# pkhungurn/talking-head-anime-4-demo

Hardware: NVIDIA H100
Metric: 512x512 RGBA frames/sec (higher is better)
Workload: dtype f16/tf32 operands (10-bit mantissa), f32 accumulate, f32 storage outside conv operands

## Files before the change

tha4_b200/csrc/conv_halo.cu:

```cuda
#include "conv.cuh"
#include "profiler.cuh"
#include "conv_tc_device.cuh"
#include <cuda.h>
#include <cstring>
#include <map>
#include <mutex>
#include <tuple>

namespace tha4 {
static long long* g_dbg_buf = nullptr;

namespace {

using namespace tc;
using namespace tcdev;

constexpr int HT_W = 8, HT_H = 16;
constexpr int HALO_W = HT_W + 2;
__host__ __device__ constexpr int halo_h(int wg) { return HT_H * wg + 2; }
__host__ __device__ constexpr int halo_rows(int wg) { return HALO_W * halo_h(wg); }
__host__ __device__ constexpr int halo_a_bytes(int rowb, int wg) { return ((halo_rows(wg) * rowb + 1023) / 1024) * 1024; }
__host__ __device__ constexpr int halo_threads(int wg) { return 128 * wg + 32; }
static_assert((HT_H * HALO_W * 64) % 1024 == 0, "second warpgroup's halo offset keeps the swizzle phase");

__host__ __device__ constexpr int halo_min_ctas(int bn, int sa, int cs, int op, int wg) {
    return wg > 1 ? (bn <= 32 ? 2 : 1) : cs > 1 || bn >= 128 ? 1 : ((sa == (op == OP_F16N ? 2 : 1) && bn <= 32) ? 4 : 2);
}
template <int BN, int SA, int SB, int CS, int OP, int XF, int WG>
__global__ void __launch_bounds__(halo_threads(WG), halo_min_ctas(BN, SA, CS, OP, WG)) conv_halo_kernel(const __grid_constant__ CUtensorMap tmA, const __grid_constant__ CUtensorMap tmB,
                                                                const __grid_constant__ CUtensorMap tmO32, const __grid_constant__ CUtensorMap tmO16,
                                                                const __grid_constant__ CUtensorMap tmR, const TcParams p) {
    static_assert(OP != OP_TF32, "halo kernel: f16 operands");
    static_assert(BN <= 128, "the accumulator of one warpgroup: BN registers per thread");
    static_assert(WG == 1 || (WG == 2 && CS == 1 && BN <= 64), "two consumer warpgroups: unsplit launches, two accumulators of at most 64 columns");
    constexpr int ROWB = op_row_bytes(OP);
    constexpr int KCE = op_kch(OP);
    constexpr int HALO_ROWS = halo_rows(WG);
    constexpr int A_BYTES = halo_a_bytes(ROWB, WG);
    constexpr int B_BYTES = BN * ROWB;
    constexpr int PRODUCER_WARP = 4 * WG;
    constexpr int EPI_BYTES = (int)(((size_t)SA * A_BYTES + (size_t)SB * B_BYTES) / WG) & ~1023;
    constexpr int NSLOT = CS == 1 ? epi_nslot(BN, EPI_BYTES) : 0;
    extern __shared__ uint8_t smem_raw[];
    uint8_t* smem = smem_raw + ((1024u - (tc::smem_u32(smem_raw) & 1023u)) & 1023u);
    uint8_t* smA = smem;
    uint8_t* smB = smem + SA * A_BYTES;
    uint64_t* bars = reinterpret_cast<uint64_t*>(smB + SB * B_BYTES);
    uint64_t* a_full = bars, *a_empty = bars + SA;
    uint64_t* b_full = bars + 2 * SA, *b_empty = b_full + SB;
    uint64_t* res_bars = b_empty + SB;
    float* xf_A = reinterpret_cast<float*>(reinterpret_cast<uint8_t*>(res_bars + 4 * WG) + ((16u - (tc::smem_u32(res_bars + 4 * WG) & 15u)) & 15u));

    const int warp = threadIdx.x >> 5, lane = threadIdx.x & 31;
    const bool dbg_on = p.dbg != nullptr && (blockIdx.x % 97) == 0 && blockIdx.y == 0 && (blockIdx.x / 97) * CS + blockIdx.z < 32;
    long long* dbg = dbg_on ? p.dbg + ((blockIdx.x / 97) * CS + blockIdx.z) * 32 : nullptr;
#define HSTAMP(role, i) do { if (dbg) dbg[(role) * 8 + (i)] = clock64(); } while (0)
    if (threadIdx.x == 0) HSTAMP(0, 0);
    int tile = blockIdx.x;
    const int tx = tile % p.tiles_x; tile /= p.tiles_x;
    const int ty = tile % p.tiles_y;
    const int n = tile / p.tiles_y;
    const int x0 = tx * HT_W, y0 = ty * (HT_H * WG);
    const int n0 = blockIdx.y * BN;
    const int split = blockIdx.z;
    const int c_per = (p.cpt + CS - 1) / CS;
    const int cb0 = split * c_per;
    const int nc = max(0, min(p.cpt, cb0 + c_per) - cb0);
    const int nb = nc * 9;

    if (threadIdx.x == 0) {
        for (int s = 0; s < SA; ++s) { mbar_init(smem_u32(a_full + s), 1); mbar_init(smem_u32(a_empty + s), 128 * WG); }
        for (int s = 0; s < SB; ++s) { mbar_init(smem_u32(b_full + s), 1); mbar_init(smem_u32(b_empty + s), 128 * WG); }
        for (int s = 0; s < 4 * WG; ++s) mbar_init(smem_u32(res_bars + s), 1);
        asm volatile("fence.mbarrier_init.release.cluster;\n" ::: "memory");
        asm volatile("prefetch.tensormap [%0];\n" :: "l"(&tmA) : "memory");
        asm volatile("prefetch.tensormap [%0];\n" :: "l"(&tmB) : "memory");
    }
    __syncthreads();
    if (threadIdx.x == 0) HSTAMP(0, 1);
    pdl_trigger();
    const int npre = p.pre_b ? min(nb, SB) : 0;
    if (warp == PRODUCER_WARP && lane == 0) {
        for (int i = 0; i < npre; ++i) {
            const uint32_t full = smem_u32(b_full + i);
            mbar_expect_tx(full, B_BYTES);
            tma_load_3d(smem_u32(smB + i * B_BYTES), &tmB, (cb0 + i / 9) * KCE, n0, i % 9, full);
        }
    }
    pdl_wait();
    if (threadIdx.x == 0) HSTAMP(0, 2);

    Acc<BN> acc;
    if (nc > 0) {
        if (warp == PRODUCER_WARP) {
            if (lane == 0) {
                int bi = 0;
                for (int ci = 0; ci < nc; ++ci) {
                    const int sa = ci % SA;
                    mbar_wait(smem_u32(a_empty + sa), ((ci / SA) & 1) ^ 1);
                    mbar_expect_tx(smem_u32(a_full + sa), HALO_ROWS * ROWB);
                    tma_load_4d(smem_u32(smA + sa * A_BYTES), &tmA, (cb0 + ci) * KCE, x0 - 1, y0 - 1, n, smem_u32(a_full + sa));
                    for (int tap = 0; tap < 9; ++tap, ++bi) {
                        if (bi < npre) continue;
                        const int sb = bi % SB;
                        mbar_wait(smem_u32(b_empty + sb), ((bi / SB) & 1) ^ 1);
                        mbar_expect_tx(smem_u32(b_full + sb), B_BYTES);
                        tma_load_3d(smem_u32(smB + sb * B_BYTES), &tmB, (cb0 + ci) * KCE, n0, tap, smem_u32(b_full + sb));
                    }
                }
            }
        } else {
            const int te = threadIdx.x;
            const int wg = WG == 1 ? 0 : te >> 7;
            constexpr int XBAR = WG == 1 ? 1 : 3;
            __half* hA = reinterpret_cast<__half*>(xf_A);
            __half* hB = hA + p.xf_C;
            const bool silu = p.xf_act == ACT_SILU || p.xf_act == ACT_SILU_FAST;
            if (XF) {
                double2* chs = reinterpret_cast<double2*>(xf_A + 2 * p.xf_C);
                xf_build_coef<128 * WG, XBAR>(p, n, te, hA, hB, chs, cb0 * KCE, (cb0 + nc) * KCE);
                if (te == 0) HSTAMP(2, 0);
            }
// ... 5 lines not shown
                if (XF) {
                    const int c0 = (cb0 + ci) * KCE;
                    constexpr int HC = ROWB / 32;
                    for (int it = te; it < 2 * HALO_ROWS; it += 128 * WG) {
                        const int row = it >> 1, half = it & 1;
                        const int hy = row / HALO_W, hx = row - hy * HALO_W;
                        const int iy = y0 - 1 + hy, ix = x0 - 1 + hx;
                        if (iy < 0 || iy >= p.inH || ix < 0 || ix >= p.inW) continue;
                        const int swz = ROWB == 128 ? (row & 7) : ((row >> 1) & 3);
                        xf_chunks<HC>(smA + sa * A_BYTES + row * ROWB, swz, half * HC, c0, p, hA, hB, silu);
                    }
                    asm volatile("fence.proxy.async.shared::cta;\n" ::: "memory");
                    asm volatile("bar.sync %0, %1;\n" :: "n"(XBAR), "n"(128 * WG) : "memory");
                    if (te == 0 && ci == nc - 1) HSTAMP(2, 2);
                }
                const uint32_t a_base = smem_u32(smA + sa * A_BYTES) + (uint32_t)(wg * HT_H * HALO_W * ROWB);
#pragma unroll
                for (int tap = 0; tap < 9; ++tap, ++bi) {
                    const int sb = bi % SB;
                    mbar_wait(smem_u32(b_full + sb), (bi / SB) & 1);
                    const int shift = (p.dy[0][tap] + 1) * HALO_W + (p.dx[0][tap] + 1);
                    const uint32_t a0 = a_base + shift * ROWB, a1 = a0 + 8 * HALO_W * ROWB;
                    const uint32_t b_addr = smem_u32(smB + sb * B_BYTES);
                    wg_fence();
#pragma unroll
                    for (int k = 0; k < ROWB / 32; ++k) {
                        const uint64_t bd = make_smem_desc_sw<ROWB>(b_addr + 32 * k);
                        const uint32_t accum = (ci > 0 || tap > 0 || k > 0) ? 1u : 0u;
                        Wgmma<BN>::f16(acc.d[0], make_desc_sbo<ROWB>(a0 + 32 * k, HALO_W * ROWB), bd, accum);
                        Wgmma<BN>::f16(acc.d[1], make_desc_sbo<ROWB>(a1 + 32 * k, HALO_W * ROWB), bd, accum);
                    }
                    wg_commit();
                    if (tap < 8) {
                        wg_wait<1>();
                        if (tap > 0) mbar_arrive(smem_u32(b_empty + (bi - 1) % SB));
                    } else {
                        wg_wait<0>();
                        mbar_arrive(smem_u32(b_empty + (bi - 1) % SB));
                        mbar_arrive(smem_u32(b_empty + bi % SB));
                        mbar_arrive(smem_u32(a_empty + sa));
                    }
                }
            }
            wg_fence_acc(acc.d[0]); wg_fence_acc(acc.d[1]);
            if (te == 0) { HSTAMP(1, 1); HSTAMP(2, 3); }
            if constexpr (WG > 1) asm volatile("bar.sync 3, 256;\n" ::: "memory");
            if (CS == 1) epi_direct<BN, HT_W, NSLOT, WG>(p, acc, smem + wg * EPI_BYTES, n, y0 + wg * HT_H, x0, n0, 0, 0, warp, lane,
                                                         &tmO32, &tmO16, &tmR, res_bars + 4 * wg, wg, EPI_BYTES);
            if (te == 0) HSTAMP(2, 4);
        }
    }
    if (CS > 1) {
        asm volatile("barrier.cluster.arrive.release.aligned;\n" ::: "memory");
        asm volatile("barrier.cluster.wait.acquire.aligned;\n" ::: "memory");
        if (threadIdx.x == 0) HSTAMP(2, 5);
        if (warp < PRODUCER_WARP && nc > 0) epi_push_partial<BN, CS>(acc, smem, split, warp, lane);
        asm volatile("barrier.cluster.arrive.release.aligned;\n" ::: "memory");
        asm volatile("barrier.cluster.wait.acquire.aligned;\n" ::: "memory");
        if (threadIdx.x == 0) HSTAMP(2, 7);
        if (warp < PRODUCER_WARP) epi_cluster_reduce<BN, CS, HT_W>(p, smem, n, y0, x0, n0, 0, split, warp, dbg);
        if (threadIdx.x == 0) HSTAMP(2, 6);
    }
    __syncthreads();
    if (threadIdx.x == 0) HSTAMP(0, 3);
#undef HSTAMP
}

typedef CUresult (*EncodeTiledFn)(CUtensorMap*, CUtensorMapDataType, cuuint32_t, void*, const cuuint64_t*, const cuuint64_t*,
                                  const cuuint32_t*, const cuuint32_t*, CUtensorMapInterleave, CUtensorMapSwizzle,
                                  CUtensorMapL2promotion, CUtensorMapFloatOOBfill);
EncodeTiledFn halo_encode() {
// ... 18 lines not shown
    auto it = g_halo_maps.find(key);
    if (it != g_halo_maps.end()) return it->second;
    CUtensorMap m;
    cuuint64_t dims[4] = {(cuuint64_t)v.C, (cuuint64_t)v.W, (cuuint64_t)v.H, (cuuint64_t)v.N};
    cuuint64_t strides[3] = {(cuuint64_t)v.ld * 2, (cuuint64_t)v.W * v.ld * 2, (cuuint64_t)v.H * v.W * v.ld * 2};
    cuuint32_t box[4] = {(cuuint32_t)op_kch(op), (cuuint32_t)HALO_W, (cuuint32_t)halo_h(wg), 1};
    cuuint32_t es[4] = {1, 1, 1, 1};
    CUresult r = halo_encode()(&m, CU_TENSOR_MAP_DATA_TYPE_FLOAT16, 4, v.p, dims, strides, box, es, CU_TENSOR_MAP_INTERLEAVE_NONE,
                               op == OP_F16N ? CU_TENSOR_MAP_SWIZZLE_64B : CU_TENSOR_MAP_SWIZZLE_128B, CU_TENSOR_MAP_L2_PROMOTION_L2_128B,
                               CU_TENSOR_MAP_FLOAT_OOB_FILL_NONE);
    THA4_REQUIRE(r == CUDA_SUCCESS, "cuTensorMapEncodeTiled(halo activation) failed: " + std::to_string((int)r));
    return g_halo_maps.emplace(key, m).first->second;
}

const CUtensorMap& halo_weight_map(const ConvWeights& cw, int bn, int op) {
    HKey key{current_device(), cw.w16, cw.cin_pad, cw.cout_pad, cw.ntaps, bn, -1, op};
    std::lock_guard<std::mutex> lock(g_halo_mu);
    auto it = g_halo_maps.find(key);
    if (it != g_halo_maps.end()) return it->second;
    CUtensorMap m;
    cuuint64_t dims[3] = {(cuuint64_t)cw.cin_pad, (cuuint64_t)cw.cout_pad, (cuuint64_t)cw.ntaps};
    cuuint64_t strides[2] = {(cuuint64_t)cw.cin_pad * 2, (cuuint64_t)cw.cout_pad * cw.cin_pad * 2};
    cuuint32_t box[3] = {(cuuint32_t)op_kch(op), (cuuint32_t)bn, 1};
    cuuint32_t es[3] = {1, 1, 1};
    CUresult r = halo_encode()(&m, CU_TENSOR_MAP_DATA_TYPE_FLOAT16, 3, cw.w16, dims, strides, box, es, CU_TENSOR_MAP_INTERLEAVE_NONE,
                               op == OP_F16N ? CU_TENSOR_MAP_SWIZZLE_64B : CU_TENSOR_MAP_SWIZZLE_128B, CU_TENSOR_MAP_L2_PROMOTION_L2_256B,
                               CU_TENSOR_MAP_FLOAT_OOB_FILL_NONE);
    THA4_REQUIRE(r == CUDA_SUCCESS, "cuTensorMapEncodeTiled(halo weights) failed: " + std::to_string((int)r));
    return g_halo_maps.emplace(key, m).first->second;
}

bool halo_store_map(const View& v, bool f16, const CUtensorMap** out) {
    const int es = f16 ? 2 : 4;
    if (!v.p || (reinterpret_cast<uintptr_t>(v.p) & 15) || ((long)v.ld * es) % 16 != 0) return false;
    HKey key{current_device(), v.p, v.N, v.H, v.W, v.C, v.ld, f16 ? -2 : -3};
    std::lock_guard<std::mutex> lock(g_halo_mu);
// ... 8 lines not shown
                                   CU_TENSOR_MAP_INTERLEAVE_NONE, f16 ? CU_TENSOR_MAP_SWIZZLE_64B : CU_TENSOR_MAP_SWIZZLE_128B,
                                   CU_TENSOR_MAP_L2_PROMOTION_NONE, CU_TENSOR_MAP_FLOAT_OOB_FILL_NONE);
        if (r != CUDA_SUCCESS) return false;
        it = g_halo_maps.emplace(key, m).first;
    }
    *out = &it->second;
    return true;
}

int g_halo_m256 = -1;

struct HaloPlan { int bn, tiles_x, tiles_y, tiles_m, tiles_n, cs, chunks, wg; };

HaloPlan halo_plan(const ConvWeights& cw, const ConvArgs& a, int op) {
    HaloPlan pl;
    pl.tiles_x = ceil_div(a.out.W, HT_W); pl.tiles_y = ceil_div(a.out.H, HT_H);
    pl.tiles_m = pl.tiles_x * pl.tiles_y * a.in.N;
    pl.chunks = cw.cin_pad / op_kch(op);
    pl.bn = (cw.cout_pad % 128 == 0) ? 128 : (cw.cout_pad % 64 == 0 ? 64 : 32);
    const int sms = num_sms();
    pl.cs = 1;
    long ctas = (long)pl.tiles_m * (cw.cout_pad / pl.bn);
    const bool m256 = g_halo_m256 > 0 || (g_halo_m256 < 0 && a.ksplit <= 1 && 8L * pl.tiles_m >= sms);
    if (a.ksplit > 1) {
        while (pl.cs * 2 <= std::min(8, a.ksplit)) pl.cs *= 2;
    } else if (a.ksplit <= 0 && ctas < sms * 13 / 16 && !m256) {
        while (pl.bn > 64 && (long)pl.tiles_m * (cw.cout_pad / pl.bn) < sms && cw.cout_pad % (pl.bn / 2) == 0) pl.bn /= 2;
        ctas = (long)pl.tiles_m * (cw.cout_pad / pl.bn);
        const int want = std::max(2, (int)((3 * sms / 2 + ctas - 1) / ctas));
        while (pl.cs < 8 && pl.cs * 2 <= want && pl.cs * 2 <= pl.chunks) pl.cs *= 2;
        while (pl.bn > 32 && (long)pl.tiles_m * (cw.cout_pad / pl.bn) * pl.cs < 96 && cw.cout_pad % (pl.bn / 2) == 0) pl.bn /= 2;
    }
    while (pl.cs > 1 && (pl.cs > pl.chunks || ceil_div(pl.chunks, ceil_div(pl.chunks, pl.cs)) != pl.cs)) pl.cs /= 2;
    pl.tiles_n = cw.cout_pad / pl.bn;
    pl.wg = 1;
    if (pl.cs == 1 && m256) {
        pl.wg = 2;
        pl.tiles_y = ceil_div(a.out.H, 2 * HT_H);
        pl.tiles_m = pl.tiles_x * pl.tiles_y * a.in.N;
        pl.bn = std::min(pl.bn, 64);
        pl.tiles_n = cw.cout_pad / pl.bn;
    }
    return pl;
}

template <int OP, int BN, int SA, int SB, int CS, int XF, int WG = 1>
void launch_halo(const CUtensorMap& ma, const CUtensorMap& mb, const CUtensorMap& mo32, const CUtensorMap& mo16, const CUtensorMap& mr, const TcParams& p, dim3 grid, cudaStream_t s) {
    constexpr int ROWB = op_row_bytes(OP);
    constexpr size_t ring = (size_t)SA * halo_a_bytes(ROWB, WG) + (size_t)SB * BN * ROWB;
    constexpr size_t smem0 = 1024 + ring + (2 * SA + 2 * SB + 4 * WG) * 8 + 16;
    static_assert(smem0 <= 227 * 1024, "shared memory budget");
    static_assert(ring / WG >= (size_t)4 * 32 * 33 * 4 + 4 * BN * 8, "epilogue scratch must fit in the pipeline buffers");
    static_assert(WG == 1 || epi_nslot(BN, (ring / WG) & ~(size_t)1023) > 0, "two warpgroups: a TMA-store staging slot each");
    static_assert(CS == 1 || ring >= (size_t)128 * BN * 4 + 128 * 8 * 4 + 128 * 4 * 4, "partial tile + statistics scratch must fit");
    const size_t smem = smem0 + (XF ? (size_t)24 * p.xf_C + 32 : 0);
    THA4_REQUIRE(smem <= 227 * 1024, "conv_halo: shared memory budget (fused input normalisation)");
    THA4_ENSURE_SMEM((conv_halo_kernel<BN, SA, SB, CS, OP, XF, WG>), smem);
    launch_pdl(conv_halo_kernel<BN, SA, SB, CS, OP, XF, WG>, grid, dim3(halo_threads(WG)), smem, s, CS, ma, mb, mo32, mo16, mr, p);
    THA4_LAUNCH_CHECK();
}

constexpr int halo_sb_wg2(int op, int bn, int sa, int sb_min) {
    const size_t a = (size_t)sa * halo_a_bytes(op_row_bytes(op), 2), b = (size_t)bn * op_row_bytes(op);
    int sb = sb_min;
    while (a + sb * b < 2 * (size_t)(epi_slot0(bn) + EPI_SLOT_BYTES)) ++sb;
    return sb;
}

template <int OP, int BN, int SA, int SBD, int SBS, int XF>
void launch_halo_cs(int cs, int wg, const CUtensorMap& ma, const CUtensorMap& mb, const CUtensorMap& mo32, const CUtensorMap& mo16, const CUtensorMap& mr, const TcParams& p, dim3 grid, cudaStream_t s) {
    constexpr int SA1 = OP == OP_F16N ? 2 : 1;
    THA4_REQUIRE(wg == 1 || (BN <= 64 && cs == 1), "conv_halo: 256-pixel tiles need an unsplit launch with N tiles of at most 64 columns");
    if constexpr (BN <= 64) {
// ... 25 lines not shown
    else if (bn == 64) launch_halo_cs<OP, 64, 2 * M, 8 * M, 3 * M, XF>(cs, wg, ma, mb, mo32, mo16, mr, p, grid, s);
    else launch_halo_cs<OP, 32, 2 * M, 9 * M, 5 * M, XF>(cs, wg, ma, mb, mo32, mo16, mr, p, grid, s);
}

bool g_use_halo = true;
bool g_tma_store = true;

}

void conv_halo_enable(bool on) { g_use_halo = on; }
void conv_halo_enable_tma_store(bool on) { g_tma_store = on; }
void conv_halo_set_m256(int mode) { g_halo_m256 = mode; }

bool conv_halo_supported(const ConvWeights& cw, const ConvArgs& a) {
    if (!g_use_halo || !conv_tc_supported(cw, a)) return false;
    if (!a.in.f16 || cw.ntaps != 9 || cw.nphase != 1 || cw.stride != 1 || cw.out_mul != 1) return false;
    for (int t = 0; t < 9; ++t)
        if (cw.dy[0][t] < -1 || cw.dy[0][t] > 1 || cw.dx[0][t] < -1 || cw.dx[0][t] > 1) return false;
    return a.in.H == a.out.H && a.in.W == a.out.W;
}

bool conv_halo_fuses_stats(const ConvWeights&, const ConvArgs&) { return true; }

void conv_halo_forward(const ConvWeights& cw, const ConvArgs& a, cudaStream_t s) {
    THA4_REQUIRE(conv_halo_supported(cw, a), "conv_halo: unsupported configuration");
    THA4_REQUIRE(a.in.C == cw.cin && a.out.C == cw.cout && a.in.N == a.out.N, "conv_halo: shapes");
    const int op = cw.cin_pad % 64 == 0 ? OP_F16 : OP_F16N;
    TcParams p{};
    p.out = a.out.p; p.outH = a.out.H; p.outW = a.out.W; p.outC = a.out.C; p.out_ld = a.out.ld;
    p.out16 = a.out16.p ? a.out16.hp() : nullptr; p.out16_ld = a.out16.ld;
    if (a.out16.p) THA4_REQUIRE(a.out16.f16 && a.out16.N == a.out.N && a.out16.H == a.out.H && a.out16.W == a.out.W && a.out16.C == a.out.C, "conv_halo: f16 output copy geometry");
    p.inH = a.in.H; p.inW = a.in.W; p.inC = a.in.C;
    if (a.nin.on) {
        const ConvNormIn& ni = a.nin;
        THA4_REQUIRE(ni.stats != nullptr && ni.gamma != nullptr && ni.beta != nullptr, "conv_halo: fused input normalisation needs statistics and affine parameters");
        THA4_REQUIRE(ni.C > 0 && ni.C <= a.in.C && ni.C % 8 == 0 && ni.C <= 1024, "conv_halo: normalised channel count");
        THA4_REQUIRE(ni.groups == 0 || (ni.C == a.in.C && ni.C % ni.groups == 0), "conv_halo: GroupNorm spans the whole input");
        p.in_stats = ni.stats; p.in_stats_ld = ni.stats_ld; p.in_stats_rep = std::max(1, ni.stats_rep); p.in_stats_rep_stride = ni.stats_rep_stride;
        p.xf_C = ni.C; p.xf_groups = ni.groups; p.xf_act = ni.act;
        p.xf_inv_cnt = 1.0 / ((double)a.in.H * a.in.W * (ni.groups == 0 ? 1 : ni.C / ni.groups));
        p.xf_gamma = ni.gamma; p.xf_beta = ni.beta; p.xf_film0 = ni.film0; p.xf_film1 = ni.film1; p.xf_film1_ld = ni.film1_ld;
    }
    p.bias = cw.bias;
    p.res = a.res.p; p.res_mode = a.res.p ? a.res_mode : RES_NONE;
    p.resH = a.res.H; p.resW = a.res.W; p.res_ld = a.res.ld;
    p.N = a.in.N; p.out_mul = 1; p.in_mul = 1;
    const HaloPlan pl = halo_plan(cw, a, op);
    p.MH = a.out.H; p.MW = a.out.W; p.tiles_x = pl.tiles_x; p.tiles_y = pl.tiles_y;
    p.pre_b = cw.dynamic ? 0 : 1;
    p.ntaps = 9; p.cpt = pl.chunks;
    if (!cw.w16) { conv_make_half(cw, s); p.pre_b = 0; }
    p.acc_scale = 1.0f / cw.w16_scale;
    for (int t = 0; t < 9; ++t) { p.dy[0][t] = cw.dy[0][t]; p.dx[0][t] = cw.dx[0][t]; }
    p.ph_oy[0] = 0; p.ph_ox[0] = 0;
    p.ksplit = 1;
    p.ws = nullptr;
    p.stats = a.out.stats; p.stats_ld = a.out.stats_ld;
    p.stats_rep = std::max(1, a.out.stats_rep); p.stats_rep_stride = a.out.stats_rep_stride;
    static const bool dbg_env = getenv("THA4_HALO_DEBUG") != nullptr;
    if (dbg_env) {
        if (!g_dbg_buf) { THA4_CUDA_CHECK(cudaMalloc(&g_dbg_buf, 32 * 32 * sizeof(long long))); }
        THA4_CUDA_CHECK(cudaMemsetAsync(g_dbg_buf, 0, 32 * 32 * sizeof(long long), s));
        p.dbg = g_dbg_buf;
    }
    ProfScope prof(PROF_CONV, s);
    prof_add_work(PROF_CONV, 2.0 * (double)p.N * p.MH * p.MW * cw.cout * cw.cin * 9, 0.0);
    const CUtensorMap& ma = halo_activation_map(a.in, op, pl.wg);
    const CUtensorMap& mb = halo_weight_map(cw, pl.bn, op);
    const CUtensorMap* mo32 = &ma;
    const CUtensorMap* mo16 = &ma;
    const CUtensorMap* mr = &ma;
    p.st_tma = 0;
    if (pl.cs == 1 && g_tma_store) {
        if (a.out.p && halo_store_map(a.out, false, &mo32)) p.st_tma |= 1;
        if (a.out16.p && halo_store_map(a.out16, true, &mo16)) p.st_tma |= 2;
        if ((p.st_tma & 1) && a.res.p && p.res_mode == RES_SAME && !a.res.f16 && a.res.N == a.out.N && a.res.H == a.out.H &&
            a.res.W == a.out.W && a.res.C >= a.out.C && halo_store_map(a.res, false, &mr)) p.st_tma |= 4;
    }
    p.vec4 = ((!cw.bias || (reinterpret_cast<uintptr_t>(cw.bias) & 15) == 0) &&
              (!a.res.p || ((reinterpret_cast<uintptr_t>(a.res.p) & 15) == 0 && a.res.ld % 4 == 0))) ? 1 : 0;
    dim3 grid(pl.tiles_m, pl.tiles_n, pl.cs);
    if (op == OP_F16) {
        if (a.nin.on) launch_halo_bn<OP_F16, 1>(pl.bn, pl.cs, pl.wg, ma, mb, *mo32, *mo16, *mr, p, grid, s);
        else launch_halo_bn<OP_F16, 0>(pl.bn, pl.cs, pl.wg, ma, mb, *mo32, *mo16, *mr, p, grid, s);
    } else {
        if (a.nin.on) launch_halo_bn<OP_F16N, 1>(pl.bn, pl.cs, pl.wg, ma, mb, *mo32, *mo16, *mr, p, grid, s);
        else launch_halo_bn<OP_F16N, 0>(pl.bn, pl.cs, pl.wg, ma, mb, *mo32, *mo16, *mr, p, grid, s);
    }
    static const bool dbg_all = dbg_env && !strcmp(getenv("THA4_HALO_DEBUG"), "2");
    if (dbg_all) {
        fprintf(stderr, "halo launch: N %d %dx%d cin %d cout %d | bn %d cs %d wg %d chunks %d grid %d x %d | xf %d groups %d act %d res %d out32 %d out16 %d st_tma %d\n",
                p.N, p.MH, p.MW, cw.cin, cw.cout, pl.bn, pl.cs, pl.wg, pl.chunks, pl.tiles_m, pl.tiles_n, a.nin.on ? 1 : 0, p.xf_groups, p.xf_act,
                p.res_mode, p.out ? 1 : 0, p.out16 ? 1 : 0, p.st_tma);
        conv_halo_debug_dump();
    }
}

void conv_halo_debug_dump() {
    if (!g_dbg_buf) return;
    std::vector<long long> h(32 * 32);
    THA4_CUDA_CHECK(cudaDeviceSynchronize());
    THA4_CUDA_CHECK(cudaMemcpy(h.data(), g_dbg_buf, h.size() * sizeof(long long), cudaMemcpyDeviceToHost));
    for (int c = 0; c < 32; ++c) {
        const long long* d = h.data() + c * 32;
        if (!d[0]) continue;
        auto rel = [&](long long v) { return v ? (long)(v - d[0]) : -1L; };
        fprintf(stderr, "halo slot %2d: init %ld pdl %ld | coef %ld a_full %ld xf_done %ld | mma_first %ld mma_commit %ld | t_full %ld epi_done %ld | bar_A %ld pushed+bar_B %ld (loads issued %ld stored %ld) reduce_done %ld | end %ld\n",
                c, rel(d[1]), rel(d[2]), rel(d[16]), rel(d[17]), rel(d[18]), rel(d[8]), rel(d[9]), rel(d[19]), rel(d[20]), rel(d[21]), rel(d[23]), rel(d[25]), rel(d[24]), rel(d[22]), rel(d[3]));
// ... 5 lines not shown
```

tha4_b200/csrc/nets.cu:

```cuda
#include "nets.cuh"
#include <algorithm>
#include <cmath>
#include <cstdlib>

namespace tha4 {

Pool::~Pool() { for (void* p : all_) cudaFree(p); }

float* Pool::alloc(size_t nfloats) {
    size_t bytes = ((nfloats * sizeof(float) + 255) / 256) * 256;
    if (bytes == 0) bytes = 256;
    Bucket& bk = buckets_[bytes];
    if (bk.next < bk.blocks.size()) return reinterpret_cast<float*>(bk.blocks[bk.next++]);
    void* p = nullptr;
    THA4_CUDA_CHECK(cudaMalloc(&p, bytes));
    bk.blocks.push_back(p);
    bk.next = bk.blocks.size();
    all_.push_back(p);
    total_ += bytes;
    return reinterpret_cast<float*>(p);
}

void Pool::reset() { for (auto& kv : buckets_) kv.second.next = 0; }

// ... 129 lines not shown
    if (want_f32) a.f = make_view(pool, N, H, W, C, stats ? &rt : nullptr);
    else {
        View v; v.N = N; v.H = H; v.W = W; v.C = C; v.ld = C;
        if (stats) {
            const int tiles = ((W + 15) / 16) * ((H + 7) / 8);
            int rep = 1;
            while (rep < stats_rep_cap() && rep * 32 <= tiles) rep *= 2;
            v.stats_rep = rep; v.stats_rep_stride = (long)N * C * 2;
            v.stats = rt.alloc_stats((size_t)rep * N * C * 2); v.stats_ld = C;
        }
        a.f = v;
    }
    if (want_f16) a.h = make_view16(pool, N, H, W, C);
    return a;
}
Tens slice_act(const Tens& a, int c0, int c) {
    Tens r;
    if (a.f.p) r.f = a.f.slice(c0, c);
    else { r.f = a.f; r.f.C = c; if (r.f.stats) r.f.stats = a.f.stats + 2 * c0; }
    if (a.h.p) r.h = a.h.slice(c0, c);
    return r;
}

ConvNormIn norm_in(const View& src_stats, const NormW& nw, int groups, int act, const float* film0 = nullptr,
                   const float* film1 = nullptr, int film1_ld = 0, int C = 0) {
    THA4_REQUIRE(src_stats.stats != nullptr, "fused normalisation: the producer did not accumulate statistics");
    ConvNormIn n;
    n.on = true; n.C = C > 0 ? C : src_stats.C; n.groups = groups; n.act = act;
    THA4_REQUIRE(nw.C == n.C, "fused normalisation: channel mismatch");
    n.gamma = nw.gamma; n.beta = nw.beta; n.film0 = film0; n.film1 = film1; n.film1_ld = film1_ld;
// ... 433 lines not shown
    rt.scratch->reset();
    float* coef = tail_coef(rt, feat, last_n_, 32);
    ImgView none{};
    tail_forward(TAIL_UNET, tail_, feat, coef, rt.strict ? ACT_SILU : ACT_SILU_FAST, image, none, outputs, s, rt.strict);
}

namespace {

struct UNetFused {
    Runtime& rt;
    const float* film1;
    int film1_total;

    void res_block(const ResBlockW& w, const Tens& x, int mode, const Tens& out) {
        rt.scratch->reset();
        THA4_REQUIRE(x.f.C == w.cin && out.f.C == w.cout && x.f.p && x.h.p, "res_block: stream tensors carry both precisions");
        const int B = x.f.N;
        const int act = ACT_SILU_FAST;
        Tens h0 = make_act(rt.scratch, rt, B, out.f.H, out.f.W, w.cout, false, true);
        Tens sk;
        if (w.has_skip) {
            sk = make_act(rt.scratch, rt, B, x.f.H, x.f.W, w.cout, true, false, false);
            if (rt.side) {
                THA4_CUDA_CHECK(cudaEventRecord(rt.ev_fork, rt.stream));
                THA4_CUDA_CHECK(cudaStreamWaitEvent(rt.side, rt.ev_fork, 0));
                cudaStream_t main_stream = rt.stream;
                rt.stream = rt.side;
                try { run_conv_tc(rt, w.skip, x.h, nullptr, sk); } catch (...) { rt.stream = main_stream; throw; }
                rt.stream = main_stream;
                THA4_CUDA_CHECK(cudaEventRecord(rt.ev_join, rt.side));
            } else {
// ... 68 lines not shown
    const int NH = 2 * L_;
    std::vector<int> hs_ch(NH);
    hs_ch[0] = mc_;
    for (int i = 0; i < L_; ++i) {
        hs_ch[2 * i + 1] = mc_ * mults_[i];
        if (i < L_ - 1) hs_ch[2 * i + 2] = mc_ * mults_[i];
    }
    std::vector<Tens> cat(NH), hs(NH);
    std::vector<int> ch_h(NH);
    for (int j = 0; j < NH; ++j) {
        const int lvl = L_ - 1 - j / 2;
        const int sp = S_ >> lvl;
        ch_h[j] = (j == 0) ? mc_ * mults_[L_ - 1] : ((j & 1) ? mc_ * mults_[lvl] : mc_ * mults_[lvl + 1]);
        const int cs = hs_ch[NH - 1 - j];
        THA4_REQUIRE(ch_h[j] + cs == up_res_[j].cin, "unet: concat plan does not match weights");
        cat[j] = make_act(P, rt, B, sp, sp, ch_h[j] + cs, true, true);
        hs[NH - 1 - j] = slice_act(cat[j], ch_h[j], cs);
    }

    run_conv_tc(rt, first_, x0, nullptr, hs[0]);
    if (rt.side) THA4_CUDA_CHECK(cudaStreamWaitEvent(s, rt.ev_join, 0));
    Tens cur = hs[0];
    for (int i = 0; i < L_; ++i) {
        if (i == L_ - 1) {
            Tens tmp = make_act(P, rt, B, cur.f.H, cur.f.W, down_res_[i].cout, true, true);
            F.res_block(down_res_[i], cur, 0, tmp);
            F.attn_block(down_attn_, tmp, hs[2 * i + 1]);
        } else {
            F.res_block(down_res_[i], cur, 0, hs[2 * i + 1]);
        }
        cur = hs[2 * i + 1];
        if (i < L_ - 1) {
            F.res_block(down_ds_[i], cur, 2, hs[2 * i + 2]);
            cur = hs[2 * i + 2];
        }
    }
    for (int j = 0; j < 4; ++j) {
        const bool last = (j == 3);
        Tens r = last ? slice_act(cat[0], 0, ch_h[0]) : make_act(P, rt, B, cur.f.H, cur.f.W, cur.f.C, true, true);
        F.res_block(mid_res_[j], cur, 0, r);
        cur = r;
        if (!last) {
            Tens a = make_act(P, rt, B, cur.f.H, cur.f.W, cur.f.C, true, true);
            F.attn_block(mid_attn_[j], cur, a);
            cur = a;
        }
    }
    Tens feat;
    for (int j = 0; j < NH; ++j) {
        const int lvl = L_ - 1 - j / 2;
        const bool second = (j & 1);
        const int co = up_res_[j].cout;
        Tens dst;
        if (!second) dst = slice_act(cat[j + 1], 0, ch_h[j + 1]);
        else dst = make_act(P, rt, B, cat[j].f.H, cat[j].f.W, co, true, true);
        if (lvl == L_ - 1) {
            Tens tmp = make_act(P, rt, B, cat[j].f.H, cat[j].f.W, co, true, true);
            F.res_block(up_res_[j], cat[j], 0, tmp);
            F.attn_block(up_attn_[second ? 1 : 0], tmp, dst);
        } else {
            F.res_block(up_res_[j], cat[j], 0, dst);
        }
        if (second) {
            if (lvl > 0) F.res_block(up_us_[L_ - 1 - lvl], dst, 1, slice_act(cat[j + 1], 0, ch_h[j + 1]));
            else feat = dst;
        }
    }
    rt.scratch->reset();
    ImgView none{};
    if (tail_.w16 != nullptr && feat.h.ld == feat.h.C) {
        View fv = feat.h;
        fv.stats = feat.f.stats; fv.stats_ld = feat.f.stats_ld; fv.stats_rep = feat.f.stats_rep; fv.stats_rep_stride = feat.f.stats_rep_stride;
        NormSpecTail ns; ns.groups = 32; ns.act = ACT_SILU_FAST; ns.gamma = last_n_.gamma; ns.beta = last_n_.beta;
        const View g0 = x0.slice(0, 4);
        tail_tc_forward(TAIL_UNET, tail_, fv, ns, image, none, outputs, s, &g0);
    } else {
        float* coef = tail_coef(rt, feat.f, last_n_, 32);
        tail_forward(TAIL_UNET, tail_, feat.f, coef, ACT_SILU_FAST, image, none, outputs, s, rt.strict);
    }
}

}
```

Before: 151.0.

## Run four-phase upsampling convs on halo kernel and drop unused fp32 activations

```diff
diff --git a/tha4_b200/csrc/conv_halo.cu b/tha4_b200/csrc/conv_halo.cu
--- a/tha4_b200/csrc/conv_halo.cu
+++ b/tha4_b200/csrc/conv_halo.cu
@@ -23,24 +23,31 @@
 __host__ __device__ constexpr int halo_threads(int wg) { return 128 * wg + 32; }
 static_assert((HT_H * HALO_W * 64) % 1024 == 0, "second warpgroup's halo offset keeps the swizzle phase");
 
-__host__ __device__ constexpr int halo_min_ctas(int bn, int sa, int cs, int op, int wg) {
-    return wg > 1 ? (bn <= 32 ? 2 : 1) : cs > 1 || bn >= 128 ? 1 : ((sa == (op == OP_F16N ? 2 : 1) && bn <= 32) ? 4 : 2);
-}
-template <int BN, int SA, int SB, int CS, int OP, int XF, int WG>
-__global__ void __launch_bounds__(halo_threads(WG), halo_min_ctas(BN, SA, CS, OP, WG)) conv_halo_kernel(const __grid_constant__ CUtensorMap tmA, const __grid_constant__ CUtensorMap tmB,
+__host__ __device__ constexpr int halo_min_ctas(int bn, int sa, int cs, int op, int wg, int ph = 1) {
+    return wg > 1 ? (bn * (ph == 4 ? 2 : 1) <= 32 ? 2 : 1) : cs > 1 || bn >= 128 ? 1 : ((sa == (op == OP_F16N ? 2 : 1) && bn <= 32) ? 4 : 2);
+}
+template <int PH>
+__host__ __device__ constexpr int halo_wtile(int j) { return PH == 1 ? j : ((j & 1) * 2 + ((j >> 1) & 1)) * 4 + (j >> 2); }
+
+template <int BN, int SA, int SB, int CS, int OP, int XF, int WG, int PH = 1>
+__global__ void __launch_bounds__(halo_threads(WG), halo_min_ctas(BN, SA, CS, OP, WG, PH)) conv_halo_kernel(const __grid_constant__ CUtensorMap tmA, const __grid_constant__ CUtensorMap tmB,
                                                                 const __grid_constant__ CUtensorMap tmO32, const __grid_constant__ CUtensorMap tmO16,
                                                                 const __grid_constant__ CUtensorMap tmR, const TcParams p) {
     static_assert(OP != OP_TF32, "halo kernel: f16 operands");
     static_assert(BN <= 128, "the accumulator of one warpgroup: BN registers per thread");
     static_assert(WG == 1 || (WG == 2 && CS == 1 && BN <= 64), "two consumer warpgroups: unsplit launches, two accumulators of at most 64 columns");
+    static_assert(PH == 1 || (PH == 4 && WG == 2 && BN <= 32), "four-phase layers: two warpgroups, two 128 x 32 accumulators each");
+    constexpr int SLABS = PH == 1 ? WG : 1;
+    constexpr int NACC = PH == 1 ? 1 : 2;
+    constexpr int TPC = PH == 1 ? 9 : 16;
     constexpr int ROWB = op_row_bytes(OP);
     constexpr int KCE = op_kch(OP);
-    constexpr int HALO_ROWS = halo_rows(WG);
-    constexpr int A_BYTES = halo_a_bytes(ROWB, WG);
+    constexpr int HALO_ROWS = halo_rows(SLABS);
+    constexpr int A_BYTES = halo_a_bytes(ROWB, SLABS);
     constexpr int B_BYTES = BN * ROWB;
     constexpr int PRODUCER_WARP = 4 * WG;
     constexpr int EPI_BYTES = (int)(((size_t)SA * A_BYTES + (size_t)SB * B_BYTES) / WG) & ~1023;
-    constexpr int NSLOT = CS == 1 ? epi_nslot(BN, EPI_BYTES) : 0;
+    constexpr int NSLOT = CS == 1 && PH == 1 ? epi_nslot(BN, EPI_BYTES) : 0;
     extern __shared__ uint8_t smem_raw[];
     uint8_t* smem = smem_raw + ((1024u - (tc::smem_u32(smem_raw) & 1023u)) & 1023u);
     uint8_t* smA = smem;
@@ -60,17 +67,17 @@
     const int tx = tile % p.tiles_x; tile /= p.tiles_x;
     const int ty = tile % p.tiles_y;
     const int n = tile / p.tiles_y;
-    const int x0 = tx * HT_W, y0 = ty * (HT_H * WG);
+    const int x0 = tx * HT_W, y0 = ty * (HT_H * SLABS);
     const int n0 = blockIdx.y * BN;
     const int split = blockIdx.z;
     const int c_per = (p.cpt + CS - 1) / CS;
     const int cb0 = split * c_per;
     const int nc = max(0, min(p.cpt, cb0 + c_per) - cb0);
-    const int nb = nc * 9;
+    const int nb = nc * TPC;
 
     if (threadIdx.x == 0) {
         for (int s = 0; s < SA; ++s) { mbar_init(smem_u32(a_full + s), 1); mbar_init(smem_u32(a_empty + s), 128 * WG); }
-        for (int s = 0; s < SB; ++s) { mbar_init(smem_u32(b_full + s), 1); mbar_init(smem_u32(b_empty + s), 128 * WG); }
+        for (int s = 0; s < SB; ++s) { mbar_init(smem_u32(b_full + s), 1); mbar_init(smem_u32(b_empty + s), PH == 1 ? 128 * WG : 128); }
         for (int s = 0; s < 4 * WG; ++s) mbar_init(smem_u32(res_bars + s), 1);
         asm volatile("fence.mbarrier_init.release.cluster;\n" ::: "memory");
         asm volatile("prefetch.tensormap [%0];\n" :: "l"(&tmA) : "memory");
@@ -84,13 +91,13 @@
         for (int i = 0; i < npre; ++i) {
             const uint32_t full = smem_u32(b_full + i);
             mbar_expect_tx(full, B_BYTES);
-            tma_load_3d(smem_u32(smB + i * B_BYTES), &tmB, (cb0 + i / 9) * KCE, n0, i % 9, full);
+            tma_load_3d(smem_u32(smB + i * B_BYTES), &tmB, (cb0 + i / TPC) * KCE, n0, halo_wtile<PH>(i % TPC), full);
         }
     }
     pdl_wait();
     if (threadIdx.x == 0) HSTAMP(0, 2);
 
-    Acc<BN> acc;
+    Acc<BN> acc[NACC];
     if (nc > 0) {
         if (warp == PRODUCER_WARP) {
             if (lane == 0) {
@@ -100,12 +107,12 @@
                     mbar_wait(smem_u32(a_empty + sa), ((ci / SA) & 1) ^ 1);
                     mbar_expect_tx(smem_u32(a_full + sa), HALO_ROWS * ROWB);
                     tma_load_4d(smem_u32(smA + sa * A_BYTES), &tmA, (cb0 + ci) * KCE, x0 - 1, y0 - 1, n, smem_u32(a_full + sa));
-                    for (int tap = 0; tap < 9; ++tap, ++bi) {
+                    for (int tap = 0; tap < TPC; ++tap, ++bi) {
                         if (bi < npre) continue;
                         const int sb = bi % SB;
                         mbar_wait(smem_u32(b_empty + sb), ((bi / SB) & 1) ^ 1);
                         mbar_expect_tx(smem_u32(b_full + sb), B_BYTES);
-                        tma_load_3d(smem_u32(smB + sb * B_BYTES), &tmB, (cb0 + ci) * KCE, n0, tap, smem_u32(b_full + sb));
+                        tma_load_3d(smem_u32(smB + sb * B_BYTES), &tmB, (cb0 + ci) * KCE, n0, halo_wtile<PH>(tap), smem_u32(b_full + sb));
                     }
                 }
             }
@@ -141,39 +148,80 @@
                     asm volatile("bar.sync %0, %1;\n" :: "n"(XBAR), "n"(128 * WG) : "memory");
                     if (te == 0 && ci == nc - 1) HSTAMP(2, 2);
                 }
-                const uint32_t a_base = smem_u32(smA + sa * A_BYTES) + (uint32_t)(wg * HT_H * HALO_W * ROWB);
+                const uint32_t a_base = smem_u32(smA + sa * A_BYTES) + (uint32_t)(SLABS > 1 ? wg * HT_H * HALO_W * ROWB : 0);
+                if constexpr (PH == 4) {
 #pragma unroll
-                for (int tap = 0; tap < 9; ++tap, ++bi) {
-                    const int sb = bi % SB;
-                    mbar_wait(smem_u32(b_full + sb), (bi / SB) & 1);
-                    const int shift = (p.dy[0][tap] + 1) * HALO_W + (p.dx[0][tap] + 1);
-                    const uint32_t a0 = a_base + shift * ROWB, a1 = a0 + 8 * HALO_W * ROWB;
-                    const uint32_t b_addr = smem_u32(smB + sb * B_BYTES);
-                    wg_fence();
+                    for (int s = 0; s < 8; ++s) {
+                        const int tap = s >> 1, px = s & 1, phase = 2 * wg + px;
+                        const int bj = ci * 16 + 2 * s + wg;
+                        const int sb = bj % SB;
+                        mbar_wait(smem_u32(b_full + sb), (bj / SB) & 1);
+                        const int shift = (p.dy[phase][tap] + 1) * HALO_W + (p.dx[phase][tap] + 1);
+                        const uint32_t a0 = a_base + shift * ROWB, a1 = a0 + 8 * HALO_W * ROWB;
+                        const uint32_t b_addr = smem_u32(smB + sb * B_BYTES);
+                        wg_fence();
 #pragma unroll
-                    for (int k = 0; k < ROWB / 32; ++k) {
-                        const uint64_t bd = make_smem_desc_sw<ROWB>(b_addr + 32 * k);
-                        const uint32_t accum = (ci > 0 || tap > 0 || k > 0) ? 1u : 0u;
-                        Wgmma<BN>::f16(acc.d[0], make_desc_sbo<ROWB>(a0 + 32 * k, HALO_W * ROWB), bd, accum);
-                        Wgmma<BN>::f16(acc.d[1], make_desc_sbo<ROWB>(a1 + 32 * k, HALO_W * ROWB), bd, accum);
+                        for (int k = 0; k < ROWB / 32; ++k) {
+                            const uint64_t bd = make_smem_desc_sw<ROWB>(b_addr + 32 * k);
+                            const uint32_t accum = (ci > 0 || tap > 0 || k > 0) ? 1u : 0u;
+                            Wgmma<BN>::f16(acc[px].d[0], make_desc_sbo<ROWB>(a0 + 32 * k, HALO_W * ROWB), bd, accum);
+                            Wgmma<BN>::f16(acc[px].d[1], make_desc_sbo<ROWB>(a1 + 32 * k, HALO_W * ROWB), bd, accum);
+                        }
+                        wg_commit();
+                        if (s < 7) {
+                            wg_wait<1>();
+                            if (s > 0) mbar_arrive(smem_u32(b_empty + (bj - 2) % SB));
+                        } else {
+                            wg_wait<0>();
+                            mbar_arrive(smem_u32(b_empty + (bj - 2) % SB));
+                            mbar_arrive(smem_u32(b_empty + sb));
+                            mbar_arrive(smem_u32(a_empty + sa));
+                        }
                     }
-                    wg_commit();
-                    if (tap < 8) {
-                        wg_wait<1>();
-                        if (tap > 0) mbar_arrive(smem_u32(b_empty + (bi - 1) % SB));
-                    } else {
-                        wg_wait<0>();
-                        mbar_arrive(smem_u32(b_empty + (bi - 1) % SB));
-                        mbar_arrive(smem_u32(b_empty + bi % SB));
-                        mbar_arrive(smem_u32(a_empty + sa));
+                } else {
+#pragma unroll
+                    for (int tap = 0; tap < 9; ++tap, ++bi) {
+                        const int sb = bi % SB;
+                        mbar_wait(smem_u32(b_full + sb), (bi / SB) & 1);
+                        const int shift = (p.dy[0][tap] + 1) * HALO_W + (p.dx[0][tap] + 1);
+                        const uint32_t a0 = a_base + shift * ROWB, a1 = a0 + 8 * HALO_W * ROWB;
+                        const uint32_t b_addr = smem_u32(smB + sb * B_BYTES);
+                        wg_fence();
+#pragma unroll
+                        for (int k = 0; k < ROWB / 32; ++k) {
+                            const uint64_t bd = make_smem_desc_sw<ROWB>(b_addr + 32 * k);
+                            const uint32_t accum = (ci > 0 || tap > 0 || k > 0) ? 1u : 0u;
+                            Wgmma<BN>::f16(acc[0].d[0], make_desc_sbo<ROWB>(a0 + 32 * k, HALO_W * ROWB), bd, accum);
+                            Wgmma<BN>::f16(acc[0].d[1], make_desc_sbo<ROWB>(a1 + 32 * k, HALO_W * ROWB), bd, accum);
+                        }
+                        wg_commit();
+                        if (tap < 8) {
+                            wg_wait<1>();
+                            if (tap > 0) mbar_arrive(smem_u32(b_empty + (bi - 1) % SB));
+                        } else {
+                            wg_wait<0>();
+                            mbar_arrive(smem_u32(b_empty + (bi - 1) % SB));
+                            mbar_arrive(smem_u32(b_empty + bi % SB));
+                            mbar_arrive(smem_u32(a_empty + sa));
+                        }
                     }
                 }
             }
-            wg_fence_acc(acc.d[0]); wg_fence_acc(acc.d[1]);
+#pragma unroll
+            for (int a = 0; a < NACC; ++a) { wg_fence_acc(acc[a].d[0]); wg_fence_acc(acc[a].d[1]); }
             if (te == 0) { HSTAMP(1, 1); HSTAMP(2, 3); }
             if constexpr (WG > 1) asm volatile("bar.sync 3, 256;\n" ::: "memory");
-            if (CS == 1) epi_direct<BN, HT_W, NSLOT, WG>(p, acc, smem + wg * EPI_BYTES, n, y0 + wg * HT_H, x0, n0, 0, 0, warp, lane,
-                                                         &tmO32, &tmO16, &tmR, res_bars + 4 * wg, wg, EPI_BYTES);
+            if constexpr (PH == 4) {
+#pragma unroll
+                for (int px = 0; px < 2; ++px) {
+                    if (px > 0) asm volatile("bar.sync 3, 256;\n" ::: "memory");
+                    epi_direct<BN, HT_W, 0, WG>(p, acc[px], smem + wg * EPI_BYTES, n, y0, x0, n0, 2 * wg + px, 0, warp, lane,
+                                                nullptr, nullptr, nullptr, nullptr, wg, EPI_BYTES);
+                }
+            } else if (CS == 1) {
+                epi_direct<BN, HT_W, NSLOT, WG>(p, acc[0], smem + wg * EPI_BYTES, n, y0 + wg * HT_H, x0, n0, 0, 0, warp, lane,
+                                                &tmO32, &tmO16, &tmR, res_bars + 4 * wg, wg, EPI_BYTES);
+            }
             if (te == 0) HSTAMP(2, 4);
         }
     }
@@ -181,7 +229,7 @@
         asm volatile("barrier.cluster.arrive.release.aligned;\n" ::: "memory");
         asm volatile("barrier.cluster.wait.acquire.aligned;\n" ::: "memory");
         if (threadIdx.x == 0) HSTAMP(2, 5);
-        if (warp < PRODUCER_WARP && nc > 0) epi_push_partial<BN, CS>(acc, smem, split, warp, lane);
+        if (warp < PRODUCER_WARP && nc > 0) epi_push_partial<BN, CS>(acc[0], smem, split, warp, lane);
         asm volatile("barrier.cluster.arrive.release.aligned;\n" ::: "memory");
         asm volatile("barrier.cluster.wait.acquire.aligned;\n" ::: "memory");
         if (threadIdx.x == 0) HSTAMP(2, 7);
@@ -230,12 +278,12 @@
 }
 
 const CUtensorMap& halo_weight_map(const ConvWeights& cw, int bn, int op) {
-    HKey key{current_device(), cw.w16, cw.cin_pad, cw.cout_pad, cw.ntaps, bn, -1, op};
+    HKey key{current_device(), cw.w16, cw.cin_pad, cw.cout_pad, cw.ntaps * cw.nphase, bn, -1, op};
     std::lock_guard<std::mutex> lock(g_halo_mu);
     auto it = g_halo_maps.find(key);
     if (it != g_halo_maps.end()) return it->second;
     CUtensorMap m;
-    cuuint64_t dims[3] = {(cuuint64_t)cw.cin_pad, (cuuint64_t)cw.cout_pad, (cuuint64_t)cw.ntaps};
+    cuuint64_t dims[3] = {(cuuint64_t)cw.cin_pad, (cuuint64_t)cw.cout_pad, (cuuint64_t)cw.ntaps * cw.nphase};
     cuuint64_t strides[2] = {(cuuint64_t)cw.cin_pad * 2, (cuuint64_t)cw.cout_pad * cw.cin_pad * 2};
     cuuint32_t box[3] = {(cuuint32_t)op_kch(op), (cuuint32_t)bn, 1};
     cuuint32_t es[3] = {1, 1, 1};
@@ -274,9 +322,15 @@
 
 HaloPlan halo_plan(const ConvWeights& cw, const ConvArgs& a, int op) {
     HaloPlan pl;
+    pl.chunks = cw.cin_pad / op_kch(op);
+    if (cw.nphase == 4) {
+        pl.tiles_x = ceil_div(a.in.W, HT_W); pl.tiles_y = ceil_div(a.in.H, HT_H);
+        pl.tiles_m = pl.tiles_x * pl.tiles_y * a.in.N;
+        pl.bn = 32; pl.tiles_n = cw.cout_pad / 32; pl.cs = 1; pl.wg = 2;
+        return pl;
+    }
     pl.tiles_x = ceil_div(a.out.W, HT_W); pl.tiles_y = ceil_div(a.out.H, HT_H);
     pl.tiles_m = pl.tiles_x * pl.tiles_y * a.in.N;
-    pl.chunks = cw.cin_pad / op_kch(op);
     pl.bn = (cw.cout_pad % 128 == 0) ? 128 : (cw.cout_pad % 64 == 0 ? 64 : 32);
     const int sms = num_sms();
     pl.cs = 1;
@@ -304,19 +358,19 @@
     return pl;
 }
 
-template <int OP, int BN, int SA, int SB, int CS, int XF, int WG = 1>
+template <int OP, int BN, int SA, int SB, int CS, int XF, int WG = 1, int PH = 1>
 void launch_halo(const CUtensorMap& ma, const CUtensorMap& mb, const CUtensorMap& mo32, const CUtensorMap& mo16, const CUtensorMap& mr, const TcParams& p, dim3 grid, cudaStream_t s) {
     constexpr int ROWB = op_row_bytes(OP);
-    constexpr size_t ring = (size_t)SA * halo_a_bytes(ROWB, WG) + (size_t)SB * BN * ROWB;
+    constexpr size_t ring = (size_t)SA * halo_a_bytes(ROWB, PH == 1 ? WG : 1) + (size_t)SB * BN * ROWB;
     constexpr size_t smem0 = 1024 + ring + (2 * SA + 2 * SB + 4 * WG) * 8 + 16;
     static_assert(smem0 <= 227 * 1024, "shared memory budget");
     static_assert(ring / WG >= (size_t)4 * 32 * 33 * 4 + 4 * BN * 8, "epilogue scratch must fit in the pipeline buffers");
-    static_assert(WG == 1 || epi_nslot(BN, (ring / WG) & ~(size_t)1023) > 0, "two warpgroups: a TMA-store staging slot each");
+    static_assert(WG == 1 || PH == 4 || epi_nslot(BN, (ring / WG) & ~(size_t)1023) > 0, "two warpgroups: a TMA-store staging slot each");
     static_assert(CS == 1 || ring >= (size_t)128 * BN * 4 + 128 * 8 * 4 + 128 * 4 * 4, "partial tile + statistics scratch must fit");
     const size_t smem = smem0 + (XF ? (size_t)24 * p.xf_C + 32 : 0);
     THA4_REQUIRE(smem <= 227 * 1024, "conv_halo: shared memory budget (fused input normalisation)");
-    THA4_ENSURE_SMEM((conv_halo_kernel<BN, SA, SB, CS, OP, XF, WG>), smem);
-    launch_pdl(conv_halo_kernel<BN, SA, SB, CS, OP, XF, WG>, grid, dim3(halo_threads(WG)), smem, s, CS, ma, mb, mo32, mo16, mr, p);
+    THA4_ENSURE_SMEM((conv_halo_kernel<BN, SA, SB, CS, OP, XF, WG, PH>), smem);
+    launch_pdl(conv_halo_kernel<BN, SA, SB, CS, OP, XF, WG, PH>, grid, dim3(halo_threads(WG)), smem, s, CS, ma, mb, mo32, mo16, mr, p);
     THA4_LAUNCH_CHECK();
 }
 
@@ -372,10 +426,16 @@
 
 bool conv_halo_supported(const ConvWeights& cw, const ConvArgs& a) {
     if (!g_use_halo || !conv_tc_supported(cw, a)) return false;
-    if (!a.in.f16 || cw.ntaps != 9 || cw.nphase != 1 || cw.stride != 1 || cw.out_mul != 1) return false;
-    for (int t = 0; t < 9; ++t)
-        if (cw.dy[0][t] < -1 || cw.dy[0][t] > 1 || cw.dx[0][t] < -1 || cw.dx[0][t] > 1) return false;
-    return a.in.H == a.out.H && a.in.W == a.out.W;
+    if (!a.in.f16 || cw.stride != 1) return false;
+    const bool four_phase = cw.nphase == 4 && cw.ntaps == 4 && cw.out_mul == 2;
+    if (!four_phase && (cw.ntaps != 9 || cw.nphase != 1 || cw.out_mul != 1)) return false;
+    for (int ph = 0; ph < cw.nphase; ++ph)
+        for (int t = 0; t < cw.ntaps; ++t)
+            if (cw.dy[ph][t] < -1 || cw.dy[ph][t] > 1 || cw.dx[ph][t] < -1 || cw.dx[ph][t] > 1) return false;
+    if (!four_phase) return a.in.H == a.out.H && a.in.W == a.out.W;
+    if (cw.cin_pad % 64 != 0 || a.ksplit > 1 || a.out.H != 2 * a.in.H || a.out.W != 2 * a.in.W) return false;
+    const HaloPlan pl = halo_plan(cw, a, OP_F16);
+    return a.ksplit == 1 || (long)pl.tiles_m * pl.tiles_n >= 64;
 }
 
 bool conv_halo_fuses_stats(const ConvWeights&, const ConvArgs&) { return true; }
@@ -402,15 +462,17 @@
     p.bias = cw.bias;
     p.res = a.res.p; p.res_mode = a.res.p ? a.res_mode : RES_NONE;
     p.resH = a.res.H; p.resW = a.res.W; p.res_ld = a.res.ld;
-    p.N = a.in.N; p.out_mul = 1; p.in_mul = 1;
+    p.N = a.in.N; p.out_mul = cw.out_mul; p.in_mul = 1;
     const HaloPlan pl = halo_plan(cw, a, op);
-    p.MH = a.out.H; p.MW = a.out.W; p.tiles_x = pl.tiles_x; p.tiles_y = pl.tiles_y;
+    p.MH = a.out.H / cw.out_mul; p.MW = a.out.W / cw.out_mul; p.tiles_x = pl.tiles_x; p.tiles_y = pl.tiles_y;
     p.pre_b = cw.dynamic ? 0 : 1;
-    p.ntaps = 9; p.cpt = pl.chunks;
+    p.ntaps = cw.ntaps; p.cpt = pl.chunks;
     if (!cw.w16) { conv_make_half(cw, s); p.pre_b = 0; }
     p.acc_scale = 1.0f / cw.w16_scale;
-    for (int t = 0; t < 9; ++t) { p.dy[0][t] = cw.dy[0][t]; p.dx[0][t] = cw.dx[0][t]; }
-    p.ph_oy[0] = 0; p.ph_ox[0] = 0;
+    for (int ph = 0; ph < cw.nphase; ++ph) {
+        p.ph_oy[ph] = cw.ph_oy[ph]; p.ph_ox[ph] = cw.ph_ox[ph];
+        for (int t = 0; t < cw.ntaps; ++t) { p.dy[ph][t] = cw.dy[ph][t]; p.dx[ph][t] = cw.dx[ph][t]; }
+    }
     p.ksplit = 1;
     p.ws = nullptr;
     p.stats = a.out.stats; p.stats_ld = a.out.stats_ld;
@@ -422,14 +484,14 @@
         p.dbg = g_dbg_buf;
     }
     ProfScope prof(PROF_CONV, s);
-    prof_add_work(PROF_CONV, 2.0 * (double)p.N * p.MH * p.MW * cw.cout * cw.cin * 9, 0.0);
-    const CUtensorMap& ma = halo_activation_map(a.in, op, pl.wg);
+    prof_add_work(PROF_CONV, 2.0 * (double)p.N * p.MH * p.MW * cw.cout * cw.cin * cw.ntaps * cw.nphase, 0.0);
+    const CUtensorMap& ma = halo_activation_map(a.in, op, cw.nphase == 1 ? pl.wg : 1);
     const CUtensorMap& mb = halo_weight_map(cw, pl.bn, op);
     const CUtensorMap* mo32 = &ma;
     const CUtensorMap* mo16 = &ma;
     const CUtensorMap* mr = &ma;
     p.st_tma = 0;
-    if (pl.cs == 1 && g_tma_store) {
+    if (pl.cs == 1 && g_tma_store && cw.nphase == 1) {
         if (a.out.p && halo_store_map(a.out, false, &mo32)) p.st_tma |= 1;
         if (a.out16.p && halo_store_map(a.out16, true, &mo16)) p.st_tma |= 2;
         if ((p.st_tma & 1) && a.res.p && p.res_mode == RES_SAME && !a.res.f16 && a.res.N == a.out.N && a.res.H == a.out.H &&
@@ -438,7 +500,10 @@
     p.vec4 = ((!cw.bias || (reinterpret_cast<uintptr_t>(cw.bias) & 15) == 0) &&
               (!a.res.p || ((reinterpret_cast<uintptr_t>(a.res.p) & 15) == 0 && a.res.ld % 4 == 0))) ? 1 : 0;
     dim3 grid(pl.tiles_m, pl.tiles_n, pl.cs);
-    if (op == OP_F16) {
+    if (cw.nphase == 4) {
+        if (a.nin.on) launch_halo<OP_F16, 32, 2, 16, 1, 1, 2, 4>(ma, mb, *mo32, *mo16, *mr, p, grid, s);
+        else launch_halo<OP_F16, 32, 2, 16, 1, 0, 2, 4>(ma, mb, *mo32, *mo16, *mr, p, grid, s);
+    } else if (op == OP_F16) {
         if (a.nin.on) launch_halo_bn<OP_F16, 1>(pl.bn, pl.cs, pl.wg, ma, mb, *mo32, *mo16, *mr, p, grid, s);
         else launch_halo_bn<OP_F16, 0>(pl.bn, pl.cs, pl.wg, ma, mb, *mo32, *mo16, *mr, p, grid, s);
     } else {
@@ -447,9 +512,9 @@
     }
     static const bool dbg_all = dbg_env && !strcmp(getenv("THA4_HALO_DEBUG"), "2");
     if (dbg_all) {
-        fprintf(stderr, "halo launch: N %d %dx%d cin %d cout %d | bn %d cs %d wg %d chunks %d grid %d x %d | xf %d groups %d act %d res %d out32 %d out16 %d st_tma %d\n",
+        fprintf(stderr, "halo launch: N %d %dx%d cin %d cout %d | bn %d cs %d wg %d chunks %d grid %d x %d | xf %d groups %d act %d res %d out32 %d out16 %d st_tma %d | phases %d\n",
                 p.N, p.MH, p.MW, cw.cin, cw.cout, pl.bn, pl.cs, pl.wg, pl.chunks, pl.tiles_m, pl.tiles_n, a.nin.on ? 1 : 0, p.xf_groups, p.xf_act,
-                p.res_mode, p.out ? 1 : 0, p.out16 ? 1 : 0, p.st_tma);
+                p.res_mode, p.out ? 1 : 0, p.out16 ? 1 : 0, p.st_tma, cw.nphase);
         conv_halo_debug_dump();
     }
 }
diff --git a/tha4_b200/csrc/nets.cu b/tha4_b200/csrc/nets.cu
--- a/tha4_b200/csrc/nets.cu
+++ b/tha4_b200/csrc/nets.cu
@@ -167,6 +167,7 @@
     if (want_f16) a.h = make_view16(pool, N, H, W, C);
     return a;
 }
+Tens f16_only(Tens a) { a.f.p = nullptr; return a; }
 Tens slice_act(const Tens& a, int c0, int c) {
     Tens r;
     if (a.f.p) r.f = a.f.slice(c0, c);
@@ -630,7 +631,9 @@
 
     void res_block(const ResBlockW& w, const Tens& x, int mode, const Tens& out) {
         rt.scratch->reset();
-        THA4_REQUIRE(x.f.C == w.cin && out.f.C == w.cout && x.f.p && x.h.p, "res_block: stream tensors carry both precisions");
+        const bool reads_f32 = mode == 2 || !w.has_skip, reads_f16 = mode != 2 || w.has_skip;
+        THA4_REQUIRE(x.f.C == w.cin && out.f.C == w.cout && (x.f.p || !reads_f32) && (x.h.p || !reads_f16),
+                     "res_block: the input lacks a precision the block reads");
         const int B = x.f.N;
         const int act = ACT_SILU_FAST;
         Tens h0 = make_act(rt.scratch, rt, B, out.f.H, out.f.W, w.cout, false, true);
@@ -729,6 +732,7 @@
         ch_h[j] = (j == 0) ? mc_ * mults_[L_ - 1] : ((j & 1) ? mc_ * mults_[lvl] : mc_ * mults_[lvl + 1]);
         const int cs = hs_ch[NH - 1 - j];
         THA4_REQUIRE(ch_h[j] + cs == up_res_[j].cin, "unet: concat plan does not match weights");
+        THA4_REQUIRE(up_res_[j].has_skip, "unet: an up ResBlock reads its concatenation through a 1x1 skip (no fp32 residual)");
         cat[j] = make_act(P, rt, B, sp, sp, ch_h[j] + cs, true, true);
         hs[NH - 1 - j] = slice_act(cat[j], ch_h[j], cs);
     }
@@ -746,13 +750,13 @@
         }
         cur = hs[2 * i + 1];
         if (i < L_ - 1) {
-            F.res_block(down_ds_[i], cur, 2, hs[2 * i + 2]);
-            cur = hs[2 * i + 2];
+            cur = down_res_[i + 1].has_skip ? f16_only(hs[2 * i + 2]) : hs[2 * i + 2];
+            F.res_block(down_ds_[i], hs[2 * i + 1], 2, cur);
         }
     }
     for (int j = 0; j < 4; ++j) {
         const bool last = (j == 3);
-        Tens r = last ? slice_act(cat[0], 0, ch_h[0]) : make_act(P, rt, B, cur.f.H, cur.f.W, cur.f.C, true, true);
+        Tens r = last ? f16_only(slice_act(cat[0], 0, ch_h[0])) : make_act(P, rt, B, cur.f.H, cur.f.W, cur.f.C, true, true);
         F.res_block(mid_res_[j], cur, 0, r);
         cur = r;
         if (!last) {
@@ -761,14 +765,15 @@
             cur = a;
         }
     }
+    const bool tc_tail = tail_.w16 != nullptr;
     Tens feat;
     for (int j = 0; j < NH; ++j) {
         const int lvl = L_ - 1 - j / 2;
         const bool second = (j & 1);
         const int co = up_res_[j].cout;
         Tens dst;
-        if (!second) dst = slice_act(cat[j + 1], 0, ch_h[j + 1]);
-        else dst = make_act(P, rt, B, cat[j].f.H, cat[j].f.W, co, true, true);
+        if (!second) dst = f16_only(slice_act(cat[j + 1], 0, ch_h[j + 1]));
+        else dst = make_act(P, rt, B, cat[j].f.H, cat[j].f.W, co, lvl > 0 || !tc_tail, true);
         if (lvl == L_ - 1) {
             Tens tmp = make_act(P, rt, B, cat[j].f.H, cat[j].f.W, co, true, true);
             F.res_block(up_res_[j], cat[j], 0, tmp);
@@ -777,13 +782,13 @@
             F.res_block(up_res_[j], cat[j], 0, dst);
         }
         if (second) {
-            if (lvl > 0) F.res_block(up_us_[L_ - 1 - lvl], dst, 1, slice_act(cat[j + 1], 0, ch_h[j + 1]));
+            if (lvl > 0) F.res_block(up_us_[L_ - 1 - lvl], dst, 1, f16_only(slice_act(cat[j + 1], 0, ch_h[j + 1])));
             else feat = dst;
         }
     }
     rt.scratch->reset();
     ImgView none{};
-    if (tail_.w16 != nullptr && feat.h.ld == feat.h.C) {
+    if (tc_tail) {
         View fv = feat.h;
         fv.stats = feat.f.stats; fv.stats_ld = feat.f.stats_ld; fv.stats_rep = feat.f.stats_rep; fv.stats_rep_stride = feat.f.stats_rep_stride;
         NormSpecTail ns; ns.groups = 32; ns.act = ACT_SILU_FAST; ns.gamma = last_n_.gamma; ns.beta = last_n_.beta;
```

Result: faster. 158.8 (median of 6 runs) (+5.2%).
